# kyle-tennison/Magnetite

Hardware: AMD Instinct MI355X
Metric: elements/sec assembly + CG iters/sec (achieved HBM GB/s), 1M-tri mesh (higher is better)
Workload: dtype f64

## Files before the change

### magnetite_amd/csrc/persist_kernel.h

```cpp
#pragma once
#include <cstring>

#include <hip/hip_runtime.h>

#include "cg_device.h"
#include "kernels.h"

namespace magk {

typedef __attribute__((address_space(1))) unsigned int gu32;
constexpr int kPersistThreads = 512, kPersistNpt = 4;

typedef __attribute__((address_space(1))) unsigned long long gu64;

__device__ inline void put_granules(unsigned long long *g, unsigned epoch, double2 v)
{
    unsigned w[4];
    __builtin_memcpy(w, &v, 16);
    const u32x4 a = {w[0], epoch, w[1], epoch}, b = {w[2], epoch, w[3], epoch};
    asm volatile("global_store_dwordx4 %0, %1, off sc1\n\tglobal_store_dwordx4 %0, %2, off offset:16 sc1" MAG_WS_DATA
                 :
                 : "v"(g), "v"(a), "v"(b)
                 : "memory");
}

__device__ inline void put_granules_at(const unsigned long long *base, uint32_t byte_off, unsigned epoch, double2 v)
{
    unsigned w[4];
    __builtin_memcpy(w, &v, 16);
    const u32x4 a = {w[0], epoch, w[1], epoch}, b = {w[2], epoch, w[3], epoch};
    asm volatile(MAG_WS_SBASE "global_store_dwordx4 %0, %1, %3 sc1\n\tglobal_store_dwordx4 %0, %2, %3 offset:16 sc1" MAG_WS_DATA
                 :
                 : "v"(byte_off), "v"(a), "v"(b), "s"(base)
                 : "memory");
}

__device__ inline bool get_granules(const unsigned long long *base, uint32_t bytes, uint32_t off, unsigned epoch,
                                    double2 &v)
{
    auto rsrc = __builtin_amdgcn_make_buffer_rsrc((void *)base, (short)0, (int)bytes, 0x00020000);
    const u32x4 a = __builtin_amdgcn_raw_buffer_load_b128(rsrc, (int)off, 0, 16);
    const u32x4 b = __builtin_amdgcn_raw_buffer_load_b128(rsrc, (int)off + 16, 0, 16);
    const bool ok = a.y == epoch && a.w == epoch && b.y == epoch && b.w == epoch;
    unsigned w[4] = {a.x, a.z, b.x, b.z};
    __builtin_memcpy(&v, w, 16);
    return ok;
}

__device__ inline double wave_sum_dpp(double v)
{
#define MAG_DPP_STEP(CTRL, ROWMASK, BOUND)                                                                           \
    {                                                                                                                  \
        const int lo = __builtin_amdgcn_update_dpp(0, __double2loint(v), CTRL, ROWMASK, 0xf, BOUND);                   \
        const int hi = __builtin_amdgcn_update_dpp(0, __double2hiint(v), CTRL, ROWMASK, 0xf, BOUND);                   \
        v += __hiloint2double(hi, lo);                                                                                 \
    }
    MAG_DPP_STEP(0x111, 0xf, true)
    MAG_DPP_STEP(0x112, 0xf, true)
    MAG_DPP_STEP(0x114, 0xf, true)
    MAG_DPP_STEP(0x118, 0xf, true)
    MAG_DPP_STEP(0x142, 0xa, false)
    MAG_DPP_STEP(0x143, 0xc, false)
#undef MAG_DPP_STEP
    return __hiloint2double(__builtin_amdgcn_readlane(__double2hiint(v), 63),
                            __builtin_amdgcn_readlane(__double2loint(v), 63));
}

[[maybe_unused]] constexpr int kStampFrom = 200, kStampTo = 1200;
constexpr int kStampPhases = 14;

template <int CTRL>
__device__ inline double dpp_move_f64(double v)
{
    const int lo = __builtin_amdgcn_update_dpp(0, __double2loint(v), CTRL, 0xf, 0xf, true);
    const int hi = __builtin_amdgcn_update_dpp(0, __double2hiint(v), CTRL, 0xf, 0xf, true);
    return __hiloint2double(hi, lo);
}

constexpr int kPersistSleep1 = 6, kPersistSleep2 = 4;
constexpr int kPersistSleepMg = 20;

template <int NH, bool OPQ = false>
__device__ inline bool persist_exchange(const PersistParams &P, int par, unsigned epoch, const int32_t (&hg)[NH],
                                        double2 (&hq)[NH], double *s_S, double2 *s_rec, double *s_chunk, double *s_part,
                                        double (&Sx)[4], unsigned long long *stamp = nullptr)
{
    int tid = threadIdx.x;
    if (OPQ) asm volatile("" : "+v"(tid));
    const int grid = gridDim.x;
    gu32 *tmo = (gu32 *)P.sync + 9;
    const unsigned long long *recb = P.recg + 8 * (int64_t)par * grid;
    const unsigned long long *qbase = P.qg + 4 * (int64_t)par * P.N;
    bool have_rec = tid >= 2 * grid, have_h[NH];
#pragma unroll
    for (int s = 0; s < NH; ++s) {
        have_h[s] = hg[s] < 0;
        hq[s] = make_double2(0.0, 0.0);
    }
    bool done = false;
    __builtin_amdgcn_s_sleep(kPersistSleep1);
    __builtin_amdgcn_s_sleep(kPersistSleep2);
#ifdef MAG_PERSIST_STAMPS
    if (stamp) stamp[0] = __builtin_amdgcn_s_memrealtime();
#endif
    bool wave_ok = false;
    unsigned spins = 0;
    for (; spins < P.spin_limit; ++spins) {
        bool ok = true;
        if (!have_rec) {
            double2 v;
            have_rec = get_granules(recb, 64u * (uint32_t)grid, 32u * (uint32_t)tid, epoch, v);
            if (have_rec) s_rec[tid] = v;
            ok = have_rec;
        }
#pragma unroll
        for (int s = 0; s < NH; ++s)
            if (!have_h[s]) {
                have_h[s] = get_granules(qbase, 32u * (uint32_t)P.N, 32u * (uint32_t)hg[s], epoch, hq[s]);
                ok &= have_h[s];
            }
        if (__all(ok ? 1 : 0)) {
            wave_ok = true;
            break;
        }
        if ((spins & 255u) == 255u) {
            const unsigned dead = (tid & 63) == 0 ? __hip_atomic_load(tmo, __ATOMIC_RELAXED, __HIP_MEMORY_SCOPE_AGENT) : 0u;
            if (__any(dead != 0u ? 1 : 0)) break;
        }
        __builtin_amdgcn_s_sleep(1);
    }
#ifdef MAG_PERSIST_STAMPS
    if (stamp) stamp[4] = __builtin_amdgcn_s_memrealtime();
#endif
    {
        constexpr int NWV = 8;
        if (blockDim.x == 64 * NWV) {
            uint32_t *s_flag = (uint32_t *)(s_chunk + 4);
            if ((tid & 63) == 0) s_flag[tid >> 6] = wave_ok ? 1u : 0u;
            __syncthreads();
            const uint4 f0 = ((const uint4 *)s_flag)[0], f1 = ((const uint4 *)s_flag)[1];
            done = (f0.x & f0.y & f0.z & f0.w & f1.x & f1.y & f1.z & f1.w) != 0u;
#ifdef MAG_PERSIST_STAMPS
            if (stamp) stamp[3] = __builtin_amdgcn_s_memrealtime();
#endif
        } else {
            done = __syncthreads_and(wave_ok ? 1 : 0) != 0;
        }
    }
#ifdef MAG_PERSIST_STAMPS
    if (stamp) {
        stamp[1] = __builtin_amdgcn_s_memrealtime();
        stamp[2] = spins + 1;
    }
#endif
    if (!done) {
        if (tid == 0) __hip_atomic_store(tmo, 1u, __ATOMIC_RELAXED, __HIP_MEMORY_SCOPE_AGENT);
        return false;
    }
    if (blockDim.x == 512) {
        const int l = tid & 63, m = 32 * (tid >> 6) + (l >> 1);
        const double2 pc = m < grid ? s_rec[2 * m + (l & 1)] : make_double2(0.0, 0.0);
        const bool two = (l & 2) != 0;
        const double k2 = two ? pc.y : pc.x, s2 = two ? pc.x : pc.y;
        double v = k2 + dpp_move_f64<0x4E>(s2);
        v += dpp_move_f64<0x114>(v);
        v += dpp_move_f64<0x118>(v);
        if ((l & 15) >= 12) s_part[(((l & 1) << 1) | ((l >> 1) & 1)) * 32 + (tid >> 6) * 4 + (l >> 4)] = v;
        __syncthreads();
        const double2 pr = ((const double2 *)(s_part + (l >> 4) * 32))[l & 15];
        double t = pr.x + pr.y;
        t += dpp_move_f64<0x111>(t);
        t += dpp_move_f64<0x112>(t);
        t += dpp_move_f64<0x114>(t);
        t += dpp_move_f64<0x118>(t);
#pragma unroll
        for (int c = 0; c < 4; ++c)
            Sx[c] = __hiloint2double(__builtin_amdgcn_readlane(__double2hiint(t), 16 * c + 15),
                                     __builtin_amdgcn_readlane(__double2loint(t), 16 * c + 15));
        return true;
    }
    if (tid < 256) {
        const int c = tid >> 6, lane = tid & 63;
        const double *rec = (const double *)s_rec;
        double v[4];
#pragma unroll
        for (int k = 0; k < 4; ++k) v[k] = lane + 64 * k < grid ? rec[4 * (lane + 64 * k) + c] : 0.0;
        double S = 0.0;
#pragma unroll
        for (int k = 0; k < 4; ++k) S = lane + 64 * k < grid ? S + v[k] : S;
        S = wave_sum_dpp(S);
        if (lane == 0) s_S[c] = S;
    }
    __syncthreads();
#pragma unroll
    for (int c = 0; c < 4; ++c) Sx[c] = s_S[c];
    return true;
}

__device__ inline void put_granules_sys(unsigned long long *g, unsigned tag, double2 v)
{
    unsigned w[4];
    __builtin_memcpy(w, &v, 16);
    const u32x4 a = {w[0], tag, w[1], tag}, b = {w[2], tag, w[3], tag};
    asm volatile("global_store_dwordx4 %0, %1, off sc0 sc1\n\tglobal_store_dwordx4 %0, %2, off offset:16 sc0 sc1" MAG_WS_DATA
                 :
                 : "v"(g), "v"(a), "v"(b)
                 : "memory");
}

__device__ inline bool get_granules_sys(const unsigned long long *base, uint32_t bytes, uint32_t off, unsigned tag,
                                        double2 &v)
{
    auto rsrc = __builtin_amdgcn_make_buffer_rsrc((void *)base, (short)0, (int)bytes, 0x00020000);
    const u32x4 a = __builtin_amdgcn_raw_buffer_load_b128(rsrc, (int)off, 0, 17);
    const u32x4 b = __builtin_amdgcn_raw_buffer_load_b128(rsrc, (int)off + 16, 0, 17);
    const bool ok = a.y == tag && a.w == tag && b.y == tag && b.w == tag;
    unsigned w[4] = {a.x, a.z, b.x, b.z};
    __builtin_memcpy(&v, w, 16);
    return ok;
}

__device__ inline void put_granules_sys_at(const uint8_t *base, uint32_t byte_off, unsigned tag, double2 v)
{
    unsigned w[4];
    __builtin_memcpy(w, &v, 16);
    const u32x4 a = {w[0], tag, w[1], tag}, b = {w[2], tag, w[3], tag};
    asm volatile(MAG_WS_SBASE "global_store_dwordx4 %0, %1, %3 sc0 sc1\n\tglobal_store_dwordx4 %0, %2, %3 offset:16 sc0 sc1" MAG_WS_DATA
                 :
                 : "v"(byte_off), "v"(a), "v"(b), "s"(base)
                 : "memory");
}

__device__ inline void publish_q(const PersistParams &P, int par, int32_t slot, uint32_t readers, unsigned tag, double2 v)
{
    const uint32_t off = 64u + 128u * (uint32_t)P.nranks + 32u * ((uint32_t)par * (uint32_t)P.n_iface + (uint32_t)slot);
    if (P.win_shared) {
        put_granules_sys_at(P.inbox[0], off, tag, v);
        return;
    }
    for (int r = 0; r < P.nranks; ++r)
        if ((readers >> r) & 1u) put_granules_sys_at(P.inbox[r], off, tag, v);
}

template <int NH>
__device__ inline bool persist_exchange_mg(const PersistParams &P, int par, unsigned tag, const int32_t (&hg)[NH],
                                           double2 (&hq)[NH], double *s_S, double2 *s_rec,
                                           [[maybe_unused]] unsigned long long *stamp = nullptr)
{
    const int tid = threadIdx.x;
    const int grid = (int)gridDim.x - P.comm_wg, R = P.nranks;
    gu32 *tmo = (gu32 *)P.sync + 9;
    uint8_t *mine = P.inbox[P.rank];
    gu32 *wtmo = (gu32 *)mine;
    auto inbox_rec = [&](int r) { return (unsigned long long *)(P.inbox[r] + 64); };
    const unsigned long long *recb = P.recg + 8 * (int64_t)par * grid;
    const unsigned long long *qbase = P.qg + 4 * (int64_t)par * P.N;
    const unsigned long long *wq =
        (const unsigned long long *)(mine + 64 + 128 * (size_t)R) + 4 * (int64_t)par * P.n_iface;
    const bool lead = blockIdx.x == 0 && !P.comm_wg;
    bool have_h[NH];
#pragma unroll
    for (int e = 0; e < NH; ++e) {
        have_h[e] = hg[e] == -1;
        hq[e] = make_double2(0.0, 0.0);
    }
    auto gave_up = [&](unsigned spins) {
        if ((spins & 255u) != 255u) return false;
        const int dead = tid == 0 && (__hip_atomic_load(tmo, __ATOMIC_RELAXED, __HIP_MEMORY_SCOPE_AGENT) != 0u ||
                                      __hip_atomic_load(wtmo, __ATOMIC_RELAXED, __HIP_MEMORY_SCOPE_SYSTEM) != 0u)
                             ? 1 : 0;
        return __syncthreads_or(dead) != 0;
    };
    auto fail = [&]() {
        if (tid == 0) __hip_atomic_store(tmo, 1u, __ATOMIC_RELAXED, __HIP_MEMORY_SCOPE_AGENT);
        if (tid < (P.win_shared ? 1 : R))
            __hip_atomic_store((gu32 *)P.inbox[tid], 1u, __ATOMIC_RELAXED, __HIP_MEMORY_SCOPE_SYSTEM);
        return false;
    };
    auto fetch_halo = [&](bool &ok, bool window) {
#pragma unroll
        for (int e = 0; e < NH; ++e)
            if (!have_h[e]) {
                if (hg[e] >= 0)
                    have_h[e] = get_granules(qbase, 32u * (uint32_t)P.N, 32u * (uint32_t)hg[e], tag, hq[e]);
                else if (window)
                    have_h[e] = get_granules_sys(wq, 32u * (uint32_t)P.n_iface, 32u * (uint32_t)(-2 - hg[e]), tag, hq[e]);
                ok &= have_h[e] || (hg[e] < 0 && !window);
            }
    };
    auto fetch_window_halo = [&]() {
        for (unsigned spins = 0; spins < P.spin_limit; ++spins) {
            bool ok = true;
            fetch_halo(ok, true);
            if (__syncthreads_and(ok ? 1 : 0)) return true;
            if (gave_up(spins)) break;
            __builtin_amdgcn_s_sleep(2);
        }
        return false;
    };
    __builtin_amdgcn_s_sleep(kPersistSleepMg);
    __builtin_amdgcn_s_sleep(kPersistSleepMg);
#ifdef MAG_PERSIST_STAMPS
    if (stamp) stamp[0] = __builtin_amdgcn_s_memrealtime();
#endif
    if (lead) {
        bool have_rec = tid >= 2 * grid, done = false;
        unsigned spins = 0;
        for (; spins < P.spin_limit; ++spins) {
            bool ok = true;
            if (!have_rec) {
                double2 v;
                have_rec = get_granules(recb, 64u * (uint32_t)grid, 32u * (uint32_t)tid, tag, v);
                if (have_rec) s_rec[tid] = v;
                ok = have_rec;
            }
            fetch_halo(ok, false);
            if (__syncthreads_and(ok ? 1 : 0)) {
                done = true;
                break;
            }
            if (gave_up(spins)) break;
            __builtin_amdgcn_s_sleep(1);
        }
        if (!done) return fail();
        if (tid < 64) {
            double S[4] = {0.0, 0.0, 0.0, 0.0};
            for (int m = tid; m < grid; m += 64) {
                const double2 a = s_rec[2 * m], b = s_rec[2 * m + 1];
                S[0] += a.x;
                S[1] += a.y;
                S[2] += b.x;
                S[3] += b.y;
            }
#pragma unroll
            for (int c = 0; c < 4; ++c) S[c] = wave_sum_dpp(S[c]);
            if (tid < 2 * (P.win_shared ? 1 : R))
                put_granules_sys(inbox_rec(tid >> 1) + 4 * (2 * ((int64_t)par * R + P.rank) + (tid & 1)), tag,
                                 (tid & 1) == 0 ? make_double2(S[0], S[1]) : make_double2(S[2], S[3]));
        }
        __syncthreads();
        bool have_w = tid >= 2 * R;
        done = false;
        for (; spins < P.spin_limit; ++spins) {
            if (!have_w) {
                double2 v;
                have_w = get_granules_sys(inbox_rec(P.rank) + 8 * (int64_t)par * R, 64u * (uint32_t)R, 32u * (uint32_t)tid,
                                          tag, v);
                if (have_w) s_rec[tid] = v;
            }
            if (__syncthreads_and(have_w ? 1 : 0)) {
                done = true;
                break;
            }
            if (gave_up(spins)) break;
            __builtin_amdgcn_s_sleep(4);
        }
        if (!done) return fail();
        if (tid < 4) {
            const double *rec = (const double *)s_rec;
            double t = 0.0;
            for (int r = 0; r < R; ++r) t += rec[4 * r + tid];
            s_S[tid] = t;
        }
        __syncthreads();
        if (tid < 2)
            put_granules(P.grec + 4 * (2 * par + tid), tag,
                         tid == 0 ? make_double2(s_S[0], s_S[1]) : make_double2(s_S[2], s_S[3]));
        return fetch_window_halo() ? true : fail();
    }
    const bool direct = P.comm_wg != 0;
    bool have_g = tid >= (direct ? 2 * R : 2), done = false;
    [[maybe_unused]] unsigned sweeps_ = 0;
    for (unsigned spins = 0; spins < P.spin_limit; ++spins) {
        ++sweeps_;
        bool ok = true;
        if (!have_g) {
            double2 v;
            have_g = direct ? get_granules_sys(inbox_rec(P.rank) + 8 * (int64_t)par * R, 64u * (uint32_t)R,
                                               32u * (uint32_t)tid, tag, v)
                            : get_granules(P.grec, 64u * 2u, 64u * (uint32_t)par + 32u * (uint32_t)tid, tag, v);
            if (have_g) s_rec[tid] = v;
            ok = have_g;
        }
        fetch_halo(ok, !P.win_shared);
        if (__syncthreads_and(ok ? 1 : 0)) {
            done = true;
            break;
        }
        if (gave_up(spins)) break;
        __builtin_amdgcn_s_sleep(2);
    }
    if (!done) return fail();
#ifdef MAG_PERSIST_STAMPS
    if (stamp) {
        stamp[1] = stamp[3] = stamp[4] = __builtin_amdgcn_s_memrealtime();
        stamp[2] = sweeps_;
    }
#endif
    if (tid < 4) {
        const double *rec = (const double *)s_rec;
        double t = rec[tid];
        if (direct) {
            t = 0.0;
            for (int r = 0; r < R; ++r) t += rec[4 * r + tid];
        }
        s_S[tid] = t;
    }
    __syncthreads();
    if (!P.win_shared) return true;
    return fetch_window_halo() ? true : fail();
}

__device__ inline void persist_comm_loop(const PersistParams &P, double *s_S, double2 *s_rec)
{
    const int tid = threadIdx.x;
    const int grid = (int)gridDim.x - 1, R = P.nranks;
    gu32 *tmo = (gu32 *)P.sync + 9;
    uint8_t *mine = P.inbox[P.rank];
    gu32 *wtmo = (gu32 *)mine;
    auto inbox_rec = [&](int r) { return (unsigned long long *)(P.inbox[r] + 64); };
    auto gave_up = [&](unsigned spins) {
        if ((spins & 255u) != 255u) return false;
        const int dead = tid == 0 && (__hip_atomic_load(tmo, __ATOMIC_RELAXED, __HIP_MEMORY_SCOPE_AGENT) != 0u ||
                                      __hip_atomic_load(wtmo, __ATOMIC_RELAXED, __HIP_MEMORY_SCOPE_SYSTEM) != 0u)
                             ? 1 : 0;
        return __syncthreads_or(dead) != 0;
    };
    auto fail = [&]() {
        if (tid == 0) __hip_atomic_store(tmo, 1u, __ATOMIC_RELAXED, __HIP_MEMORY_SCOPE_AGENT);
        if (tid < R) __hip_atomic_store((gu32 *)P.inbox[tid], 1u, __ATOMIC_RELAXED, __HIP_MEMORY_SCOPE_SYSTEM);
    };
    int par = 0;
    unsigned tag = P.tag_base + 1u;
    double target = P.tol, bb = 0.0;
#ifdef MAG_PERSIST_STAMPS
    unsigned long long cs_[4] = {0, 0, 0, 0}, cn_ = 0;
#endif
    for (long long j = 0;; ++j) {
#ifdef MAG_PERSIST_STAMPS
        const bool cst_ = tid == 0 && j >= kStampFrom && j < kStampTo;
        unsigned long long ct0_ = 0, ct1_ = 0, ct2_ = 0, ct3_ = 0;
        if (cst_) ct0_ = __builtin_amdgcn_s_memrealtime();
#endif
        const unsigned long long *recb = P.recg + 8 * (int64_t)par * grid;
        bool have_rec = tid >= 2 * grid, done = false;
        unsigned spins = 0;
        for (; spins < P.spin_limit; ++spins) {
            if (!have_rec) {
                double2 v;
                have_rec = get_granules(recb, 64u * (uint32_t)grid, 32u * (uint32_t)tid, tag, v);
                if (have_rec) s_rec[tid] = v;
            }
            if (__syncthreads_and(have_rec ? 1 : 0)) {
                done = true;
                break;
            }
            if (gave_up(spins)) break;
        }
        if (!done) return fail();
#ifdef MAG_PERSIST_STAMPS
        if (cst_) ct1_ = __builtin_amdgcn_s_memrealtime();
#endif
        if (tid < 64) {
            double S[4] = {0.0, 0.0, 0.0, 0.0};
            for (int m = tid; m < grid; m += 64) {
                const double2 a = s_rec[2 * m], b = s_rec[2 * m + 1];
                S[0] += a.x;
                S[1] += a.y;
                S[2] += b.x;
                S[3] += b.y;
            }
#pragma unroll
            for (int c = 0; c < 4; ++c) S[c] = wave_sum_dpp(S[c]);
            if (tid < 2 * R)
                put_granules_sys(inbox_rec(tid >> 1) + 4 * (2 * ((int64_t)par * R + P.rank) + (tid & 1)), tag,
                                 (tid & 1) == 0 ? make_double2(S[0], S[1]) : make_double2(S[2], S[3]));
        }
        __syncthreads();
#ifdef MAG_PERSIST_STAMPS
        if (cst_) ct2_ = __builtin_amdgcn_s_memrealtime();
#endif
        bool have_w = tid >= 2 * R;
        done = false;
        for (; spins < P.spin_limit; ++spins) {
            if (!have_w) {
                double2 v;
                have_w = get_granules_sys(inbox_rec(P.rank) + 8 * (int64_t)par * R, 64u * (uint32_t)R, 32u * (uint32_t)tid,
                                          tag, v);
                if (have_w) s_rec[tid] = v;
            }
            if (__syncthreads_and(have_w ? 1 : 0)) {
                done = true;
                break;
            }
            if (gave_up(spins)) break;
            __builtin_amdgcn_s_sleep(1);
        }
        if (!done) return fail();
#ifdef MAG_PERSIST_STAMPS
        if (cst_) {
            ct3_ = __builtin_amdgcn_s_memrealtime();
            cs_[0] += ct1_ - ct0_;
            cs_[1] += ct2_ - ct1_;
            cs_[2] += ct3_ - ct2_;
            ++cn_;
        }
#endif
        if (tid < 4) {
            const double *rec = (const double *)s_rec;
            double t = 0.0;
            for (int r = 0; r < R; ++r) t += rec[4 * r + tid];
            s_S[tid] = t;
        }
        __syncthreads();
        const double rr = s_S[0];
        if (j == 0) {
            bb = rr;
            target = P.stop_mode == 2 ? P.tol * sqrt(bb) : P.tol;
        }
        const double cost = P.stop_mode == 1 ? fabs(rr) : sqrt(rr);
        const long long it_done = j - 1;
        if ((j == 0 && bb == 0.0) || (it_done >= 1 && cost <= target) || !(fabs(rr) <= 1.79769313486231570e308) ||
            it_done >= P.max_iter) {
#ifdef MAG_PERSIST_STAMPS
            if (tid == 0 && P.stamps) {
                unsigned long long *o = P.stamps + (size_t)grid * (kStampPhases + 1);
                for (int k = 0; k < 3; ++k) o[k] = cs_[k];
                o[kStampPhases] = cn_;
            }
#endif
            return;
        }
        __syncthreads();
        par ^= 1;
        ++tag;
    }
}

constexpr int kPersistPartDoubles = 128;
template <bool OPQ = false>
__device__ inline void persist_block_sum(double (&acc)[4], double *s_part, [[maybe_unused]] unsigned long long *sub = nullptr)
{
    int tx = threadIdx.x;
    if (OPQ) asm volatile("" : "+v"(tx));
    const int l = tx & 63;
    const bool odd = (l & 1) != 0, two = (l & 2) != 0;
    const double ka = odd ? acc[2] : acc[0], kb = odd ? acc[3] : acc[1];
    const double sa = odd ? acc[0] : acc[2], sb = odd ? acc[1] : acc[3];
    const double a = ka + dpp_move_f64<0xB1>(sa), b = kb + dpp_move_f64<0xB1>(sb);
    const double k2 = two ? b : a, s2 = two ? a : b;
    double v = k2 + dpp_move_f64<0x4E>(s2);
    v += dpp_move_f64<0x114>(v);
    v += dpp_move_f64<0x118>(v);
    if ((l & 15) >= 12) s_part[(((l & 1) << 1) | ((l >> 1) & 1)) * 32 + (tx >> 6) * 4 + (l >> 4)] = v;
#ifdef MAG_PERSIST_STAMPS
    if (sub) sub[0] = __builtin_amdgcn_s_memrealtime();
#endif
    __syncthreads();
#ifdef MAG_PERSIST_STAMPS
    if (sub) sub[1] = __builtin_amdgcn_s_memrealtime();
#endif
    if (tx < 64) {
        const double2 pr = ((const double2 *)(s_part + (l >> 4) * 32))[l & 15];
        double t = pr.x + pr.y;
        t += dpp_move_f64<0x111>(t);
        t += dpp_move_f64<0x112>(t);
        t += dpp_move_f64<0x114>(t);
        t += dpp_move_f64<0x118>(t);
#pragma unroll
        for (int c = 0; c < 4; ++c)
            acc[c] = __hiloint2double(__builtin_amdgcn_readlane(__double2hiint(t), 16 * c + 15),
                                      __builtin_amdgcn_readlane(__double2loint(t), 16 * c + 15));
    }
}

constexpr int kPersistRegs = 5;
constexpr int kPersistWeights = 6;
constexpr int kPersistBlockEntries = 6;
constexpr int kPersistNh = 2;

#ifdef MAG_PERSIST_STAMPS
#define MAG_STAMP(k)                                                                                                   \
    if (stamping) {                                                                                                    \
        const unsigned long long now_ = __builtin_amdgcn_s_memrealtime();                                              \
        stamp_sum[k] += now_ - stamp_last;                                                                             \
        stamp_last = now_;                                                                                             \
    }
#else
#define MAG_STAMP(k)
#endif

template <int N>
struct PackedFlags {
    static_assert(N <= 4, "one byte per node slot");
    uint32_t v = 0;
    __device__ uint32_t operator[](int s) const { return (v >> (8 * s)) & 0xffu; }
    __device__ void set(int s, uint32_t f) { v = (v & ~(0xffu << (8 * s))) | ((f & 0xffu) << (8 * s)); }
};

__device__ inline double uniform_f64(double v)
{
    return __hiloint2double(__builtin_amdgcn_readfirstlane(__double2hiint(v)),
                            __builtin_amdgcn_readfirstlane(__double2loint(v)));
}

template <int NH>
__device__ inline void persist_single_workgroup(double *s_S, double (&Sx)[4], double2 (&hq)[NH])
{
    __syncthreads();
#pragma unroll
    for (int c = 0; c < 4; ++c) Sx[c] = uniform_f64(s_S[c]);
#pragma unroll
    for (int e = 0; e < NH; ++e) hq[e] = make_double2(0.0, 0.0);
    __syncthreads();
}

__device__ inline PersistParams persist_case_params(PersistParams P)
{
    const int64_t c = (int64_t)blockIdx.y;
    P.bP += c * P.N;
    P.x += c * P.N;
    P.qg += 8 * c * P.N;
    P.recg += 16 * c * (int64_t)gridDim.x;
    P.sync += 16 * c;
    P.st += c;
    if (c != 0) P.hist_len = 0;
    return P;
}

__device__ inline PersistParams persist_variant_operator(PersistParams P)
{
    const int64_t c = (int64_t)blockIdx.y;
    P.xyP += c * P.N;
    P.halo_xy += c * P.var_halo_stride;
    P.kblocks += c * P.var_kb_stride;
    P.ovf_rec += c * P.var_ovf_stride;
    P.c0 = P.var_mat[3 * c + 0];
    P.nu = P.var_mat[3 * c + 1];
    P.h = P.var_mat[3 * c + 2];
    return P;
}

constexpr int persist_walk_group(int B, bool MG, int EBM, bool ONE, int NPT)
{
    if (EBM == 0 || MG || ONE || NPT != 4) return 0;
    return EBM == 2 && B == 512 ? 2 : 3;
}

template <int B, bool MG, int THREADS, int EBM, bool ONE = false, int NPTX = 0, bool VAR = false, bool LC = false>
__global__ void __launch_bounds__(THREADS) k_cg_persist(const PersistParams Pk)
{
    static_assert(!(LC && MG), "load cases run on one GPU");
    static_assert(LC || !VAR, "variants are laid out as load cases");
    PersistParams Pc;
    if constexpr (LC) Pc = persist_case_params(Pk);
    if constexpr (VAR) Pc = persist_variant_operator(Pc);
    const PersistParams &P = LC ? Pc : Pk;
    constexpr int NPT = NPTX ? NPTX : kPersistNpt;
    constexpr bool EB = EBM != 0, OV = EBM == 2;
    constexpr bool OPQ = OV || (EB && !MG && B == 256);
    constexpr int SB = NPT * THREADS / B - 1;
    extern __shared__ __attribute__((aligned(16))) double2 smem[];
    const int tid = threadIdx.x;
    const int cap = P.cap, maxh = P.maxh;
    const int capx = OV ? B : cap;
    const int tile_words = capx + cap + maxh + B;
    double2 *s_rec = smem + (size_t)(NPT * THREADS / B) * tile_words;
    double *s_red = (double *)(s_rec + 2 * 256);
    double *s_S = s_red + 4 * (THREADS / 64);
    double *s_chunk = s_S + 4;
    double *s_part = s_chunk + 4 * 32;
    [[maybe_unused]] double2 *s_pool = (double2 *)(s_part + kPersistPartDoubles) + (MG ? NPT * THREADS / 4 : 0);
    auto t_loc = [&](int s) { return __builtin_amdgcn_readfirstlane((s * THREADS + tid) / B); };
    auto t_lt = [&](int s) { return (s * THREADS + tid) % B; };
    auto t_xy = [&](int s) { return smem + (size_t)t_loc(s) * tile_words; };

    const int cgrid = (int)gridDim.x - (MG ? P.comm_wg : 0);
    if (MG && P.comm_wg && (int)blockIdx.x == cgrid) {
        persist_comm_loop(P, s_S, s_rec);
        return;
    }
    constexpr int NH = kPersistNh;
    const unsigned tag0 = (MG ? P.tag_base : 0u) + 1u;
    int32_t deg[NPT], ent[NPT];
    [[maybe_unused]] uint32_t *s_opk = (uint32_t *)(s_part + kPersistPartDoubles);
    const int32_t node_base = __builtin_amdgcn_readfirstlane(((MG ? P.t0 : 0) + (int32_t)blockIdx.x * P.tiles_per_wg) * B);
    auto node_of = [&](int s) { return node_base + s * THREADS + tid; };
    int32_t hg[NH], hloc[NH];
    PackedFlags<NPT> flags;
    [[maybe_unused]] uint32_t ovpk[(NPT + 1) / 2] = {};
    [[maybe_unused]] int32_t ovmax[NPT] = {};
    uint32_t w[NPT][kPersistRegs];
    int64_t ell_off[NPT];
    double2 r[NPT], q[NPT];

    double acc[4] = {0.0, 0.0, 0.0, 0.0};
#pragma unroll
    for (int s = 0; s < NPT; ++s) {
        const int l = t_loc(s), lt = t_lt(s);
        const int32_t t = (MG ? P.t0 : 0) + blockIdx.x * P.tiles_per_wg + l;
        double2 *xy = t_xy(s), *pim = xy + capx, *hr = pim + cap, *xs = hr + maxh;
        if (MG) s_opk[s * THREADS + tid] = 0xffffffffu;
        deg[s] = 0;
        ent[s] = 0;
        flags.set(s, 3);
        ell_off[s] = 0;
        r[s] = q[s] = make_double2(0.0, 0.0);
#pragma unroll
        for (int k = 0; k < kPersistRegs; ++k) w[s][k] = 0xffffffffu;
        if (!(l < P.tiles_per_wg && t < (MG ? P.t1 : P.T))) continue;
        const TileMeta tm = P.meta[t];
        const int64_t nd = (int64_t)t * B + lt;
        flags.set(s, 8);
        if (nd < P.N) {
            const double2 b = P.bP[nd];
            r[s] = make_double2(-b.x, -b.y);
            xy[lt] = EB ? make_double2(0.0, 0.0) : P.xyP[nd];
            const uint32_t mk = P.maskP[nd];
            flags.set(s, flags[s] | 16u | (mk & 7u));
            if (!(mk & 8u)) flags.set(s, flags[s] & ~4u);
            acc[0] = fma(b.y, b.y, fma(b.x, b.x, acc[0]));
        } else {
            xy[lt] = make_double2(0.0, 0.0);
            flags.set(s, flags[s] | 3u);
        }
        pim[lt] = make_double2(0.0, 0.0);
        xs[lt] = make_double2(0.0, 0.0);
        deg[s] = tm.deg;
        ent[s] = __builtin_amdgcn_readfirstlane(tm.ent);
        ell_off[s] = tm.ell_off + lt;
#pragma unroll
        for (int k = 0; k < kPersistRegs; ++k)
            if (k < deg[s]) w[s][k] = P.ell16[ell_off[s] + (int64_t)k * B];
        {
            const int32_t t_first = (MG ? P.t0 : 0) + blockIdx.x * P.tiles_per_wg, t_end = MG ? P.t1 : P.T;
            const bool short_rows = OV || tm.ent <= 2 * kPersistRegs;
            auto remap = [&](uint32_t e) -> uint32_t {
                if (e == 0xffffu) return e;
                const uint32_t lid = e & 0xfffu;
                uint32_t slot = (uint32_t)(SB * tile_words) + lid;
                if (short_rows && lid >= (uint32_t)B) {
                    const int32_t g = P.halo_g[tm.hoff + (int32_t)(lid - B)];
                    const int32_t ot = g / B, ol = ot - t_first;
                    if (ol >= 0 && ol < P.tiles_per_wg && ot < t_end) slot = (uint32_t)((SB + ol - l) * tile_words + (g - ot * B));
                }
                return slot | (e & 0x8000u);
            };
#pragma unroll
            for (int k = 0; k < kPersistRegs; ++k)
                if (k < deg[s]) w[s][k] = remap(w[s][k] & 0xffffu) | (remap(w[s][k] >> 16) << 16);
            if (OV) {
                int32_t cnt = 0;
                uint32_t off = 0;
                if (tid == 0 && s == 0) {
                    s_pool[0] = make_double2(0.0, 0.0);
                    s_pool[1] = make_double2(0.0, __hiloint2double(0, SB * tile_words));
                }
                if (nd < P.N) {
                    constexpr int NBk = kPersistBlockEntries;
                    const uint32_t info = P.row_info[nd];
                    const int32_t n = (int32_t)(info & 63u), nblk = (info & 0x40u) ? n - 1 : n;
                    if (info & 0x40u) flags.set(s, flags[s] | 32u);
                    const int32_t g0 = P.ovf_off[nd];
                    cnt = nblk > NBk ? nblk - NBk : 0;
                    off = 1u + (uint32_t)(g0 - P.ovf_off[(int64_t)t_first * B]);
                    const double2 *src = (const double2 *)P.ovf_rec + 2 * (int64_t)g0;
                    for (int32_t k = 0; k < cnt; ++k) {
                        const double2 a = src[2 * k];
                        double2 b = src[2 * k + 1];
                        b.y = __hiloint2double(0, (int)(remap((uint32_t)__double2loint(b.y) & 0xfffu) & 0x7fffu));
                        s_pool[2 * (off + (uint32_t)k)] = a;
                        s_pool[2 * (off + (uint32_t)k) + 1] = b;
                    }
                    if (!(info & 0x40u) && n > NBk) {
                        const uint32_t ww = P.ell16[ell_off[s] + (int64_t)((n - 1) >> 1) * B];
                        const uint32_t last = remap(((n - 1) & 1) ? (ww >> 16) : (ww & 0xffffu)) & 0x7fffu;
                        constexpr int kw = (NBk - 1) >> 1;
                        w[s][kw] = ((NBk - 1) & 1) ? ((w[s][kw] & 0xffffu) | (last << 16)) : ((w[s][kw] & 0xffff0000u) | last);
                    }
                }
                ovpk[s >> 1] |= ((off & 0xfffu) | ((uint32_t)cnt << 12)) << (16 * (s & 1));
                int32_t m = 0;
                for (int32_t c = 1; c <= 15; ++c)
                    if (__any(cnt >= c ? 1 : 0)) m = c;
                ovmax[s] = __builtin_amdgcn_readfirstlane(m);
            }
        }
        if (EB) {
            constexpr int NBk = kPersistBlockEntries;
            static_assert(NBk + 1 <= 2 * kPersistRegs, "entry NB is looked at in the registers");
            const uint32_t e0 = w[s][0] & 0xffffu, eN = (NBk & 1) ? (w[s][NBk >> 1] >> 16) : (w[s][NBk >> 1] & 0xffffu);
            if (!OV && tm.ent > NBk && !(eN & 0x8000u) && (eN & 0x7fffu) == (e0 & 0x7fffu)) flags.set(s, flags[s] | 32u);
            ring_pad_entries<kPersistRegs, NBk, 0x7fffu>(w[s], tm.ent);
        }
        if ((flags[s] & 20) == 20) put_granules(P.qg + 4 * nd, tag0, make_double2(0.0, 0.0));
        if (MG && (flags[s] & 16)) {
            const int32_t osl = P.own_qslot[nd];
            if (osl >= 0) {
                uint32_t ord = 0;
                if (!P.win_shared) ord = P.iface_readers[osl];
                asm volatile("" : "+v"(ord));
                s_opk[s * THREADS + tid] = (uint32_t)osl | (ord << 24);
                flags.set(s, flags[s] | 64u);
                publish_q(P, 0, osl, ord, tag0, make_double2(0.0, 0.0));
            }
        }
    }
    {
        const int32_t t_first = (MG ? P.t0 : 0) + blockIdx.x * P.tiles_per_wg, t_end = MG ? P.t1 : P.T;
        int32_t cg[NH], cl[NH];
#pragma unroll
        for (int e = 0; e < NH; ++e) {
            cg[e] = -1;
            cl[e] = 0;
            int32_t rem = tid + THREADS * e;
            for (int l = 0; l < P.tiles_per_wg && t_first + l < t_end; ++l) {
                const TileMeta tm = P.meta[t_first + l];
                if (rem < tm.nh) {
                    const int32_t g = P.halo_g[tm.hoff + rem];
                    const int32_t ot = g / B, ol = ot - t_first;
                    const bool sibling = (OV || tm.ent <= 2 * kPersistRegs) && ol >= 0 && ol < P.tiles_per_wg && ot < t_end;
                    if (!sibling) {
                        cg[e] = g;
                        cl[e] = l * tile_words + rem;
                    }
                    break;
                }
                rem -= tm.nh;
            }
        }
        int32_t *s_cnt = (int32_t *)s_red;
        int2 *s_list = (int2 *)s_rec;
        constexpr int NW8 = THREADS / 64;
        int32_t pos[NH];
#pragma unroll
        for (int e = 0; e < NH; ++e) {
            const unsigned long long live = __ballot(cg[e] >= 0);
            pos[e] = __builtin_amdgcn_mbcnt_hi((unsigned)(live >> 32), __builtin_amdgcn_mbcnt_lo((unsigned)live, 0u));
            if ((tid & 63) == 0) s_cnt[e * NW8 + (tid >> 6)] = __popcll(live);
        }
        __syncthreads();
        int32_t total = 0;
#pragma unroll
        for (int e = 0; e < NH; ++e) {
            int32_t base = 0;
            for (int k = 0; k < e * NW8 + (tid >> 6); ++k) base += s_cnt[k];
            if (cg[e] >= 0) s_list[base + pos[e]] = make_int2(cg[e], cl[e]);
        }
        for (int k = 0; k < NH * NW8; ++k) total += s_cnt[k];
        __syncthreads();
#pragma unroll
        for (int e = 0; e < NH; ++e) {
            hg[e] = -1;
            hloc[e] = 0;
            const int32_t c = tid + THREADS * e;
            if (c < total) {
                const int2 ent2 = s_list[c];
                hg[e] = ent2.x;
                hloc[e] = ent2.y;
                const int32_t l = ent2.y / tile_words, rem = ent2.y - l * tile_words;
                const TileMeta tm = P.meta[t_first + l];
                double2 *xy = smem + (size_t)l * tile_words;
                if (!EB) xy[B + rem] = P.halo_xy[tm.hoff + rem];
                const double2 hb = P.bP[hg[e]];
                xy[capx + cap + rem] = make_double2(-hb.x, -hb.y);
                xy[capx + B + rem] = make_double2(0.0, 0.0);
                if (MG) {
                    const int32_t hs = P.halo_qslot[tm.hoff + rem];
                    if (hs >= 0) hg[e] = -2 - hs;
                }
            }
        }
        __syncthreads();
    }
    if (blockIdx.x == 0 && tid == 0) acc[1] = 1.0;
    persist_block_sum<OPQ>(acc, s_part);
    int par = 0;
    unsigned epoch = tag0;
    constexpr bool single_wg = ONE && !MG;
    if (tid < 2)
        put_granules(P.recg + 4 * (2 * ((int64_t)par * cgrid + blockIdx.x) + tid), epoch,
                     tid == 0 ? make_double2(acc[0], acc[1]) : make_double2(acc[2], acc[3]));
    if (single_wg && tid < 2) ((double2 *)s_S)[tid] = tid == 0 ? make_double2(acc[0], acc[1]) : make_double2(acc[2], acc[3]);
    double2 hq[NH];
    double Sx[4] = {0.0, 0.0, 0.0, 0.0};
    if (single_wg)
        persist_single_workgroup<NH>(s_S, Sx, hq);
    else if (MG ? !persist_exchange_mg<NH>(P, par, epoch, hg, hq, s_S, s_rec)
                : !persist_exchange<NH, OPQ>(P, par, epoch, hg, hq, s_S, s_rec, s_chunk, s_part, Sx))
        return;

    const double c0 = P.c0, nu = P.nu, h = P.h;
    constexpr int NCW = kPersistWeights;
    constexpr int NB = kPersistBlockEntries;
    constexpr bool BLOCKS = EB;
    constexpr int WG = persist_walk_group(B, MG, EBM, ONE, NPT);
    constexpr int NKB = BLOCKS ? 3 * NB : NCW;
    double wgt[NPT][NKB];
    const double kappa = uniform_f64(0.5 * (h - nu) * c0);
    if (BLOCKS) {
#pragma unroll
        for (int s = 0; s < NPT; ++s) {
            const bool live = (flags[s] & 24) == 24;
#pragma unroll
            for (int c = 0; c < NKB; ++c) wgt[s][c] = live ? P.kblocks[(int64_t)c * P.kb_stride + node_of(s)] : 0.0;
        }
#pragma unroll
        for (int s = 0; s < NPT; ++s)
#pragma unroll
            for (int c = 0; c < NKB; ++c) asm volatile("" : "+v"(wgt[s][c]));
    } else {
#pragma unroll
        for (int s = 0; s < NPT; ++s) {
#pragma unroll
            for (int c = 0; c < NKB; ++c) wgt[s][c] = 0.0;
            if (!(flags[s] & 8)) continue;
            const double2 *xy = t_xy(s);
            const int32_t nent = __builtin_amdgcn_readfirstlane(ent[s]);
            if (nent > 0)
                ring_weights<kPersistRegs, NCW, 0x7fffu>(w[s], nent, xy - SB * tile_words, xy[t_lt(s)], c0,
                                                         *reinterpret_cast<double(*)[NCW]>(&wgt[s][0]));
        }
    }
    constexpr bool QL = EB;
    bool all_live = true;
#pragma unroll
    for (int s = 0; s < NPT; ++s) all_live = all_live && (flags[s] & 8) != 0;
    all_live = __builtin_amdgcn_readfirstlane(__syncthreads_and(all_live ? 1 : 0)) != 0;
    double target = P.tol, bb = 0.0;
    long long j = 0;
    int verdict = 0;
    double cost = 0.0;
    const bool reporter = blockIdx.x == 0 && tid == 0;
    if (reporter) {
        s_chunk[0] = __builtin_inf();
        ((long long *)s_chunk)[1] = 0;
    }
#ifdef MAG_PERSIST_STAMPS
    unsigned long long *stamp_sum = (unsigned long long *)(s_chunk + 16);
    unsigned long long &stamp_last = stamp_sum[kStampPhases], &stamp_iters = stamp_sum[kStampPhases + 1];
    if (tid == 0)
        for (int k = 0; k < kStampPhases + 2; ++k) stamp_sum[k] = 0;
#endif
    for (;;) {
#ifdef MAG_PERSIST_STAMPS
        const bool stamping = tid == 0 && j >= kStampFrom && j < kStampTo;
        if (stamping) {
            stamp_last = __builtin_amdgcn_s_memrealtime();
            ++stamp_iters;
        }
#endif
        const double S0 = MG ? uniform_f64(s_S[0]) : Sx[0], S1 = MG ? uniform_f64(s_S[1]) : Sx[1],
                     S2 = MG ? uniform_f64(s_S[2]) : Sx[2], S3 = MG ? uniform_f64(s_S[3]) : Sx[3];
        if (j == 0) {
            bb = S0;
            target = uniform_f64(P.stop_mode == 2 ? P.tol * sqrt(bb) : P.tol);
        }
        const double rr = S0;
        const double alpha = uniform_f64(rr / S1);
        const double beta = uniform_f64(fma(alpha * alpha, S3, fma(2.0 * alpha, S2, rr)) / rr);
        cost = uniform_f64(P.stop_mode == 1 ? fabs(rr) : sqrt(rr));
        const long long it_done = j - 1;
        if (reporter && it_done >= 1 && it_done - 1 < P.hist_len) P.hist[it_done - 1] = cost;
        if (j == 0 && bb == 0.0) {
            verdict = 1;
            cost = 0.0;
            break;
        }
        if (reporter && it_done >= 1 && cost < s_chunk[0]) {
            s_chunk[0] = cost;
            ((long long *)s_chunk)[1] = it_done;
        }
        if (it_done >= 1 && cost <= target) verdict = 1;
        else if (!(fabs(rr) <= 1.79769313486231570e308)) verdict = 3;
        else if (it_done >= P.max_iter) verdict = 2;
        if (verdict) break;

        const bool xnow = !(beta != 0.0) || !(fabs(beta) <= 1.79769313486231570e308);
        if (xnow) {
#pragma unroll
            for (int s = 0; s < NPT; ++s) {
                if (!(flags[s] & 8)) continue;
                const int lt = t_lt(s);
                double2 *xy = t_xy(s), *pim = xy + capx, *xs = pim + cap + maxh;
                const double2 po = pim[lt];
                double2 xo = xs[lt];
                xo.x = fma(alpha, po.x, xo.x);
                xo.y = fma(alpha, po.y, xo.y);
                xs[lt] = xo;
            }
        }
        auto update_slot = [&](int s) {
            const int lt = t_lt(s);
            double2 *xy = t_xy(s), *pim = xy + capx;
            const double2 po = pim[lt];
            const double2 qv = QL ? xy[lt] : q[s];
            double2 pn;
            r[s].x = fma(alpha, qv.x, r[s].x);
            r[s].y = fma(alpha, qv.y, r[s].y);
            pn.x = fma(beta, po.x, -r[s].x);
            pn.y = fma(beta, po.y, -r[s].y);
            pim[lt] = pn;
        };
        if (all_live) {
#pragma unroll
            for (int s = 0; s < NPT; ++s) update_slot(s);
        } else {
#pragma unroll
            for (int s = 0; s < NPT; ++s)
                if (flags[s] & 8) update_slot(s);
        }
#pragma unroll
        for (int e = 0; e < NH; ++e)
            if (hg[e] != -1) {
                double2 *hbase = smem + hloc[e];
                double2 hrv = hbase[capx + cap], hpv = hbase[capx + B];
                hrv.x = fma(alpha, hq[e].x, hrv.x);
                hrv.y = fma(alpha, hq[e].y, hrv.y);
                hpv.x = fma(beta, hpv.x, -hrv.x);
                hpv.y = fma(beta, hpv.y, -hrv.y);
                hbase[capx + cap] = hrv;
                hbase[capx + B] = hpv;
            }
        MAG_STAMP(0)
        __syncthreads();
        MAG_STAMP(1)

#pragma unroll
        for (int c = 0; c < 4; ++c) acc[c] = 0.0;
        if (EB || MG) {
#pragma unroll
            for (int s = 0; s < NPT; ++s)
#pragma unroll
                for (int k = 0; k < (EB ? (kPersistBlockEntries + 1) / 2 : kPersistRegs); ++k) asm volatile("" : "+v"(w[s][k]));
        }
        if (OV) {
#pragma unroll
            for (int i = 0; i < (NPT + 1) / 2; ++i) asm volatile("" : "+v"(ovpk[i]));
        }
#pragma unroll
        for (int s = 0; s < NPT; ++s) {
            if (((tid >> 8) & 1) && s >= NPT / 2) __builtin_amdgcn_s_setprio(1);
            if (OV && ovmax[s] > 0) __builtin_amdgcn_s_setprio(2);
            else if (OV && !(((tid >> 8) & 1) && s >= NPT / 2)) __builtin_amdgcn_s_setprio(0);
            if (!(flags[s] & 8)) continue;
            const int lt = t_lt(s);
            const double2 *xy = t_xy(s), *pim = xy + capx;
            const double2 ca = xy[lt], pa = pim[lt];
            double fx = 0.0, fy = 0.0;
            {
                const int32_t nent = __builtin_amdgcn_readfirstlane(ent[s]);
                if (nent > 0) {
                    const uint32_t toff = (uint32_t)(SB * tile_words);
                    if (OV) {
                        const uint32_t oc = (ovpk[s >> 1] >> (16 * (s & 1))) & 0xffffu;
                        ring_walk_blocks_ovf<kPersistRegs, NB, 0x7fffu, WG>(
                            w[s], pim - SB * tile_words, pa, kappa, (flags[s] & 32u) != 0,
                            *reinterpret_cast<const double(*)[3 * NB]>(&wgt[s][0]), s_pool, oc & 0xfffu, oc >> 12, ovmax[s], fx, fy);
                    } else if (BLOCKS)
                        ring_walk_blocks<kPersistRegs, NB, 0x7fffu, WG>(w[s], pim - SB * tile_words, pa, kappa, (flags[s] & 32u) != 0,
                                                                        *reinterpret_cast<const double(*)[3 * NB]>(&wgt[s][0]), fx, fy);
                    else
                        ring_walk_cached<kPersistRegs, NCW, 0x7fffu>(w[s], P.ell16 + ell_off[s], B, nent, xy - SB * tile_words, pim - SB * tile_words,
                                                                     ca, pa, c0, nu, h, *reinterpret_cast<const double(*)[NCW]>(&wgt[s][0]),
                                                                     fx, fy, toff);
                }
            }
            if ((flags[s] & 1) || !(flags[s] & 16)) fx = 0.0;
            if ((flags[s] & 2) || !(flags[s] & 16)) fy = 0.0;
            const double2 qn = make_double2(fx, fy);
            if (QL) t_xy(s)[lt] = qn;
            else q[s] = qn;
            if ((flags[s] & 20) == 20)
                put_granules_at(P.qg, 32u * ((uint32_t)(par ^ 1) * (uint32_t)P.N + (uint32_t)node_of(s)), epoch + 1, qn);
            if (MG && (flags[s] & 64u)) {
                const uint32_t opk = s_opk[s * THREADS + tid];
                publish_q(P, par ^ 1, (int32_t)(opk & 0xffffffu), opk >> 24, epoch + 1, qn);
            }
            acc[0] = fma(r[s].y, r[s].y, fma(r[s].x, r[s].x, acc[0]));
            acc[1] = fma(pa.y, fy, fma(pa.x, fx, acc[1]));
            acc[2] = fma(r[s].y, fy, fma(r[s].x, fx, acc[2]));
            acc[3] = fma(fy, fy, fma(fx, fx, acc[3]));
        }
        __builtin_amdgcn_s_setprio(0);
        MAG_STAMP(2)
#ifdef MAG_PERSIST_STAMPS
        unsigned long long *sub_ = stamp_sum + kStampPhases + 8;
        persist_block_sum<OPQ>(acc, s_part, stamping ? sub_ : nullptr);
#else
        persist_block_sum<OPQ>(acc, s_part);
#endif
        par ^= 1;
        ++epoch;
        ++j;
        if (tid < 2)
            put_granules(P.recg + 4 * (2 * ((int64_t)par * cgrid + blockIdx.x) + tid), epoch,
                         tid == 0 ? make_double2(acc[0], acc[1]) : make_double2(acc[2], acc[3]));
        if (single_wg && tid < 2) ((double2 *)s_S)[tid] = tid == 0 ? make_double2(acc[0], acc[1]) : make_double2(acc[2], acc[3]);
#ifdef MAG_PERSIST_STAMPS
        if (stamping) {
            const unsigned long long now_ = __builtin_amdgcn_s_memrealtime();
            stamp_sum[8] += sub_[0] - stamp_last;
            stamp_sum[9] += sub_[1] - sub_[0];
            stamp_sum[10] += now_ - sub_[1];
            sub_[2] = now_;
        }
#endif
        if (!xnow) {
            const double ab = uniform_f64(alpha / beta);
            auto x_slot = [&](int s) {
                const int lt = t_lt(s);
                double2 *xy = t_xy(s), *pim = xy + capx, *xs = pim + cap + maxh;
                const double2 pj = pim[lt], rv = r[s];
                double2 xo = xs[lt];
                xo.x = fma(ab, pj.x + rv.x, xo.x);
                xo.y = fma(ab, pj.y + rv.y, xo.y);
                xs[lt] = xo;
            };
            if (all_live) {
#pragma unroll
                for (int s = 0; s < NPT; ++s) x_slot(s);
            } else {
#pragma unroll
                for (int s = 0; s < NPT; ++s)
                    if (flags[s] & 8) x_slot(s);
            }
        }
#ifdef MAG_PERSIST_STAMPS
        if (stamping) stamp_sum[11] += __builtin_amdgcn_s_memrealtime() - sub_[2];
#endif
        MAG_STAMP(3)
#ifdef MAG_PERSIST_STAMPS
        unsigned long long *xs_ = stamp_sum + kStampPhases + 2;
        if (stamping) xs_[0] = xs_[1] = xs_[2] = xs_[3] = xs_[4] = 0;
        if (single_wg)
            persist_single_workgroup<NH>(s_S, Sx, hq);
        else if (MG ? !persist_exchange_mg<NH>(P, par, epoch, hg, hq, s_S, s_rec, stamping ? xs_ : nullptr)
                    : !persist_exchange<NH, OPQ>(P, par, epoch, hg, hq, s_S, s_rec, s_chunk, s_part, Sx, stamping ? xs_ : nullptr))
            return;
        if (stamping) {
            stamp_sum[4] += xs_[0] - stamp_last;
            stamp_sum[5] += xs_[1] - xs_[0];
            const unsigned long long end_ = __builtin_amdgcn_s_memrealtime();
            stamp_sum[6] += end_ - xs_[1];
            stamp_sum[7] += xs_[2];
            stamp_sum[12] += xs_[3] - xs_[4];
            stamp_sum[13] += end_ - xs_[3];
        }
#else
        if (single_wg)
            persist_single_workgroup<NH>(s_S, Sx, hq);
        else if (MG ? !persist_exchange_mg<NH>(P, par, epoch, hg, hq, s_S, s_rec)
                    : !persist_exchange<NH, OPQ>(P, par, epoch, hg, hq, s_S, s_rec, s_chunk, s_part, Sx))
            return;
#endif
    }
#ifdef MAG_PERSIST_STAMPS
    if (tid == 0 && P.stamps) {
        unsigned long long *o = P.stamps + (size_t)blockIdx.x * (kStampPhases + 1);
        for (int k = 0; k < kStampPhases; ++k) o[k] = stamp_sum[k];
        o[kStampPhases] = stamp_iters;
    }
#endif
    int tid_x = tid;
    if (WG) asm volatile("" : "+v"(tid_x));
#pragma unroll
    for (int s = 0; s < NPT; ++s)
        if ((flags[s] & 24) == 24) P.x[node_base + s * THREADS + tid_x] = (t_xy(s) + capx + cap + maxh)[t_lt(s)];
    if (blockIdx.x == 0 && tid == 0) {
        FusedState *st = P.st;
        st->bb = bb;
        st->target = target;
        st->iterations = j - 1 < 0 ? 0 : j - 1;
        st->final_cost = cost;
        st->converged = verdict == 1 ? 1 : 0;
        st->breakdown = verdict == 3 ? 1 : 0;
        st->best_cost = s_chunk[0];
        st->best_iter = ((long long *)s_chunk)[1];
        st->done = 1;
    }
}

typedef void (*PersistKernel)(const PersistParams);
#define MAG_PERSIST_ROW_KERNEL(MEMBERS_, B_, MG_, EBM_, ONE_, NPTX_)                                                              \
    if (sh.B == B_ && sh.mg == MG_ && sh.ebm == EBM_ && sh.one == ONE_ && sh.nptx == NPTX_)                                       \
        return k_cg_persist<B_, MG_, 512, EBM_, ONE_, NPTX_, MEMBERS_ == PERSIST_VARIANTS, MEMBERS_ != PERSIST_SINGLE>;

}
```

Measured before the change: 34.66 million.

## Prefetch halo granules with buffer loads before spin sleep in persistent exchange

Rewrites the persistent CG exchange spin loop to use raw buffer loads with out-of-range offsets as done-markers, replacing per-entry branching on have flags. Halo loads are issued before the sleep so their latency overlaps the wait, and wave-uniform liveness checks skip loads entirely. The initial sleep constants are also raised. This adds coherence assumptions about buffer-load caching (aux 16 flag) and hardcodes NH==2.

```diff
diff --git a/magnetite_amd/csrc/persist_kernel.h b/magnetite_amd/csrc/persist_kernel.h
--- a/magnetite_amd/csrc/persist_kernel.h
+++ b/magnetite_amd/csrc/persist_kernel.h
@@ -77,7 +77,7 @@
     return __hiloint2double(hi, lo);
 }
 
-constexpr int kPersistSleep1 = 6, kPersistSleep2 = 4;
+constexpr int kPersistSleep1 = 8, kPersistSleep2 = 6;
 constexpr int kPersistSleepMg = 20;
 
 template <int NH, bool OPQ = false>
@@ -91,13 +91,44 @@
     gu32 *tmo = (gu32 *)P.sync + 9;
     const unsigned long long *recb = P.recg + 8 * (int64_t)par * grid;
     const unsigned long long *qbase = P.qg + 4 * (int64_t)par * P.N;
-    bool have_rec = tid >= 2 * grid, have_h[NH];
+    const uint32_t rec_bytes = 64u * (uint32_t)grid, q_bytes = 32u * (uint32_t)P.N;
+    const auto rsrc_rec = __builtin_amdgcn_make_buffer_rsrc((void *)recb, (short)0, (int)rec_bytes, 0x00020000);
+    const auto rsrc_q = __builtin_amdgcn_make_buffer_rsrc((void *)qbase, (short)0, (int)q_bytes, 0x00020000);
+    int tq = tid;
+    asm volatile("" : "+v"(tq));
+    uint32_t orec = 32u * (uint32_t)tq, oh[NH];
 #pragma unroll
     for (int s = 0; s < NH; ++s) {
-        have_h[s] = hg[s] < 0;
+        int32_t h = hg[s];
+        asm volatile("" : "+v"(h));
+        oh[s] = h < 0 ? q_bytes : 32u * (uint32_t)h;
         hq[s] = make_double2(0.0, 0.0);
     }
+    auto tags_ok = [&](const u32x4 &a, const u32x4 &b) { return a.y == epoch && a.w == epoch && b.y == epoch && b.w == epoch; };
+    auto value_of = [](const u32x4 &a, const u32x4 &b) {
+        const unsigned w[4] = {a.x, a.z, b.x, b.z};
+        double2 v;
+        __builtin_memcpy(&v, w, 16);
+        return v;
+    };
+    static_assert(NH == 2, "the halo registers below are written out for two entries");
+    const bool live_rec = __any(orec < rec_bytes ? 1 : 0) != 0, live_h0 = __any(oh[0] != q_bytes ? 1 : 0) != 0,
+               live_h1 = __any(oh[1] != q_bytes ? 1 : 0) != 0;
+    const u32x4 zero4 = {0u, 0u, 0u, 0u};
+    u32x4 h0a = zero4, h0b = zero4, h1a = zero4, h1b = zero4;
+    auto issue_halo = [&]() {
+        if (live_h0) {
+            h0a = __builtin_amdgcn_raw_buffer_load_b128(rsrc_q, (int)oh[0], 0, 16);
+            h0b = __builtin_amdgcn_raw_buffer_load_b128(rsrc_q, (int)oh[0] + 16, 0, 16);
+        }
+        if (live_h1) {
+            h1a = __builtin_amdgcn_raw_buffer_load_b128(rsrc_q, (int)oh[1], 0, 16);
+            h1b = __builtin_amdgcn_raw_buffer_load_b128(rsrc_q, (int)oh[1] + 16, 0, 16);
+        }
+        __builtin_amdgcn_sched_barrier(0);
+    };
     bool done = false;
+    issue_halo();
     __builtin_amdgcn_s_sleep(kPersistSleep1);
     __builtin_amdgcn_s_sleep(kPersistSleep2);
 #ifdef MAG_PERSIST_STAMPS
@@ -106,19 +137,26 @@
     bool wave_ok = false;
     unsigned spins = 0;
     for (; spins < P.spin_limit; ++spins) {
-        bool ok = true;
-        if (!have_rec) {
-            double2 v;
-            have_rec = get_granules(recb, 64u * (uint32_t)grid, 32u * (uint32_t)tid, epoch, v);
-            if (have_rec) s_rec[tid] = v;
-            ok = have_rec;
-        }
-#pragma unroll
-        for (int s = 0; s < NH; ++s)
-            if (!have_h[s]) {
-                have_h[s] = get_granules(qbase, 32u * (uint32_t)P.N, 32u * (uint32_t)hg[s], epoch, hq[s]);
-                ok &= have_h[s];
-            }
+        u32x4 ra = zero4, rb = zero4;
+        if (live_rec) {
+            ra = __builtin_amdgcn_raw_buffer_load_b128(rsrc_rec, (int)orec, 0, 16);
+            rb = __builtin_amdgcn_raw_buffer_load_b128(rsrc_rec, (int)orec + 16, 0, 16);
+        }
+        __builtin_amdgcn_sched_barrier(0);
+        const bool got_rec = orec < rec_bytes && tags_ok(ra, rb);
+        if (got_rec) s_rec[tid] = value_of(ra, rb);
+        orec = got_rec ? rec_bytes : orec;
+        bool ok = orec >= rec_bytes;
+#pragma unroll
+        for (int s = 0; s < NH; ++s) {
+            const u32x4 &a = s ? h1a : h0a, &b = s ? h1b : h0b;
+            const bool got = oh[s] != q_bytes && tags_ok(a, b);
+            const double2 v = value_of(a, b);
+            hq[s].x = got ? v.x : hq[s].x;
+            hq[s].y = got ? v.y : hq[s].y;
+            oh[s] = got ? q_bytes : oh[s];
+            ok &= oh[s] == q_bytes;
+        }
         if (__all(ok ? 1 : 0)) {
             wave_ok = true;
             break;
@@ -127,6 +165,7 @@
             const unsigned dead = (tid & 63) == 0 ? __hip_atomic_load(tmo, __ATOMIC_RELAXED, __HIP_MEMORY_SCOPE_AGENT) : 0u;
             if (__any(dead != 0u ? 1 : 0)) break;
         }
+        issue_halo();
         __builtin_amdgcn_s_sleep(1);
     }
 #ifdef MAG_PERSIST_STAMPS
```

Result: faster. 35.68 million, median of 6 (+2.9%).
